# microsoft/rl-offline-simulation

Hardware: AMD Instinct MI355X
Metric: simulated steps/sec (node), 10M logged transitions x 4096 rollouts (higher is better)
Workload: dtype f64

## Files before the change

include/offsim.h:

```cpp
#ifndef OFFSIM_H
#define OFFSIM_H

#include <stdint.h>

#ifdef __cplusplus
extern "C" {
#endif

#define OFFSIM_OK 0
#define OFFSIM_EINVAL (-1)
#define OFFSIM_EHIP (-2)
#define OFFSIM_EUNSUPPORTED (-3)

#define OFFSIM_F32 0
#define OFFSIM_F64 1
#define OFFSIM_F16 2

#define OFFSIM_REJECT_DEFAULT 0
#define OFFSIM_REJECT_NEVER 1

#define OFFSIM_PROB_F64 0
#define OFFSIM_PROB_F32 1

#define OFFSIM_ST_OK 0
// ... 1 lines not shown
#define OFFSIM_ST_NO_INIT 2
#define OFFSIM_ST_KEYERROR 3
#define OFFSIM_ST_INACTIVE 4
#define OFFSIM_ST_PROTOCOL 5

typedef struct offsim_table {
    int64_t N;
    int32_t n_slots;
    int32_t nA;
    int32_t plog_dtype;
    int32_t r_dtype;
    const uint32_t *seg_off;
    const void *p_log;
    const int32_t *a;
    const void *r;
    const int32_t *z_next;
    const uint8_t *done;
    const int32_t *orig_idx;
    int64_t N0;
    const int32_t *init_slot;
    const int32_t *init_orig;
    int64_t max_seg;
    int64_t min_seg;
} offsim_table;

typedef struct offsim_rollouts {
    int32_t R;
    uint64_t *rng;
    uint32_t *cursor;
    uint32_t *init_cursor;
    int32_t *cur_slot;
    const uint32_t *perm;
    int64_t perm_stride;
    const uint32_t *init_perm;
    int64_t init_stride;
    int32_t rng_kind;
} offsim_rollouts;
#define OFFSIM_STREAM_PCG64 0
#define OFFSIM_STREAM_PHILOX 1

const char *offsim_last_error(void);
int offsim_version(void);
int offsim_device_count(void);


int64_t offsim_group_scratch_bytes(int64_t N, int32_t n_slots);
int offsim_group_by_state(const int32_t *slot, int64_t N, int32_t n_slots, uint32_t *seg_off ,
                          int32_t *order , void *scratch, void *stream);

int offsim_gather_rows(const void *src, const int32_t *order, int64_t N, int32_t row_bytes, void *dst, void *stream);


int offsim_seed_streams(const uint64_t *seeds, int32_t R, uint64_t *rng_out , void *stream);

int offsim_shuffle_queues(const offsim_table *t, const uint64_t *seeds, int32_t n_perm, uint32_t *perm_out,
                          uint32_t *init_perm_out, void *stream);

int offsim_env_reset(const offsim_table *t, offsim_rollouts *ro, const uint8_t *mask, int32_t *out_init_row,
                     void *stream);


int offsim_step_batch(const offsim_table *t, offsim_rollouts *ro, const void *p_new, int32_t prob_mode,
                      int32_t reject_mode, int32_t advance, int32_t *out_row, int32_t *out_status,
                      uint32_t *out_popped, void *stream);

#define OFFSIM_MAILBOX_MAX_ACTIONS 24
#define OFFSIM_SERVER_CMD_STEP 1
#define OFFSIM_SERVER_CMD_POP_ONE 2
#define OFFSIM_SERVER_CMD_EXIT 3
#define OFFSIM_SERVER_CMD_RESET 4
#define OFFSIM_SERVER_STARTING 1
#define OFFSIM_SERVER_RUNNING 2
#define OFFSIM_SERVER_EXITED 3
typedef struct offsim_step_mailbox {
    uint32_t seq_in;
    uint32_t cmd;
    int32_t reject_mode;
    uint32_t reserved0;
    double p_head[5];
    uint32_t reserved1;
    uint32_t seq_in2;
    double p_tail[OFFSIM_MAILBOX_MAX_ACTIONS - 5];
    uint32_t reserved2[2];
    uint32_t seq_out;
    int32_t row;
    int32_t status;
    uint32_t popped;
    uint32_t state;
    uint32_t reserved3[3];
} offsim_step_mailbox;
int offsim_host_alloc(int64_t bytes, void **host_ptr);
int offsim_host_free(void *host_ptr);
int offsim_step_server_start(const offsim_table *t, offsim_rollouts *ro, offsim_step_mailbox *mailbox, int32_t prob_mode,
                             uint32_t idle_polls, void *stream);
#define OFFSIM_SERVER_GONE 1
#define OFFSIM_SERVER_ANSWER_SECONDS 10.0
int offsim_step_server_call(offsim_step_mailbox *mailbox, const void *p_new, int32_t n_actions, int32_t prob_mode, uint32_t cmd,
                            int32_t reject_mode, uint64_t max_spins, int32_t *out3);

int offsim_env_set_state(offsim_rollouts *ro, const int32_t *slot, const uint8_t *mask, void *stream);

typedef struct {
    const void *src;
    void *dst;
    int64_t row_bytes;
    int32_t zero_if_not_ok;
// ... 246 lines not shown
```

rl-offline-simulation_amd/_lib.py:

```python
import ctypes as C
import os

_HERE = os.path.dirname(os.path.abspath(__file__))
LIB_PATH = os.environ.get("OFFSIM_LIB") or os.path.join(_HERE, "csrc", "liboffsim_hip.so")

OK = 0
EINVAL, EHIP, EUNSUPPORTED = -1, -2, -3
F32, F64, F16 = 0, 1, 2
REJECT_DEFAULT, REJECT_NEVER = 0, 1
STREAM_PCG64, STREAM_PHILOX = 0, 1
STREAMS_A, STREAMS_B, STREAMS_C = 0, 1, 2
PROB_F64, PROB_F32 = 0, 1
ST_OK, ST_EXHAUSTED, ST_NO_INIT, ST_KEYERROR, ST_INACTIVE, ST_PROTOCOL = 0, 1, 2, 3, 4, 5

_vp, _i32, _i64, _u8 = C.c_void_p, C.c_int32, C.c_int64, C.c_uint8


class Table(C.Structure):
    _fields_ = [("N", _i64), ("n_slots", _i32), ("nA", _i32), ("plog_dtype", _i32), ("r_dtype", _i32),
                ("seg_off", _vp), ("p_log", _vp), ("a", _vp), ("r", _vp), ("z_next", _vp), ("done", _vp),
                ("orig_idx", _vp), ("N0", _i64), ("init_slot", _vp), ("init_orig", _vp), ("max_seg", _i64), ("min_seg", _i64)]


class Rollouts(C.Structure):
# ... 61 lines not shown
                ("x_dtype", _i32), ("dO", _i32), ("x_start", _vp), ("x_next", _vp), ("x_init", _vp), ("v_next", _vp), ("v_init", _vp)]


class CollectPPOOut(C.Structure):
    _fields_ = [("value", _vp), ("logp", _vp), ("final_value", _vp), ("v_trunc", _vp)]


PPO_ACTOR, PPO_CRITIC = 0, 1
PPO_MAX_BLOCKS = 256


def ppo_update_work_doubles(P):
    return PPO_MAX_BLOCKS * 8 + 8 + PPO_MAX_BLOCKS * ((P + 1) // 2)


class PPONet(C.Structure):
    _fields_ = [("n_layers", _i32), ("activation", _i32), ("layers_host", C.POINTER(MLPLayer)), ("slope", C.c_float), ("reserved", _i32)]


class PPOBatchC(C.Structure):
    _fields_ = [("obs", _vp), ("x_dtype", _i32), ("dO", _i32), ("act", _vp), ("adv", _vp), ("logp", _vp), ("ret", _vp), ("valid", _vp),
                ("M", _i64)]


class PPOAdam(C.Structure):
    _fields_ = [("m", _vp), ("v", _vp), ("t", _vp), ("lr", C.c_double)]


MAILBOX_MAX_ACTIONS = 24
SERVER_CMD_STEP, SERVER_CMD_POP_ONE, SERVER_CMD_EXIT, SERVER_CMD_RESET = 1, 2, 3, 4
SERVER_STARTING, SERVER_RUNNING, SERVER_EXITED = 1, 2, 3
SERVER_GONE = 1
SERVER_ANSWER_SECONDS = 10.0


class StepMailbox(C.Structure):
    _fields_ = [("seq_in", C.c_uint32), ("cmd", C.c_uint32), ("reject_mode", _i32), ("reserved0", C.c_uint32), ("p_head", C.c_double * 5),
                ("reserved1", C.c_uint32), ("seq_in2", C.c_uint32), ("p_tail", C.c_double * (MAILBOX_MAX_ACTIONS - 5)),
                ("reserved2", C.c_uint32 * 2), ("seq_out", C.c_uint32), ("row", _i32), ("status", _i32), ("popped", C.c_uint32),
                ("state", C.c_uint32), ("reserved3", C.c_uint32 * 3)]


TD_QLEARN, TD_EXPSARSA = 1, 2
BEHAVIOUR_FIXED, BEHAVIOUR_EPS_GREEDY, BEHAVIOUR_SOFT_GREEDY = 0, 1, 2

SIGNATURES = {
    "offsim_last_error": (C.c_char_p, []),
    "offsim_version": (C.c_int, []),
    "offsim_device_count": (C.c_int, []),
    "offsim_group_scratch_bytes": (_i64, [_i64, _i32]),
    "offsim_group_by_state": (C.c_int, [_vp, _i64, _i32, _vp, _vp, _vp, _vp]),
    "offsim_gather_rows": (C.c_int, [_vp, _vp, _i64, _i32, _vp, _vp]),
    "offsim_seed_streams": (C.c_int, [_vp, _i32, _vp, _vp]),
    "offsim_shuffle_queues": (C.c_int, [C.POINTER(Table), _vp, _i32, _vp, _vp, _vp]),
    "offsim_env_reset": (C.c_int, [C.POINTER(Table), C.POINTER(Rollouts), _vp, _vp, _vp]),
    "offsim_env_set_state": (C.c_int, [C.POINTER(Rollouts), _vp, _vp, _vp]),
    "offsim_vector_gather": (C.c_int, [_vp, _vp, _vp, C.c_int32, _vp, C.c_int32, _vp, _vp]),
    "offsim_vector_step": (C.c_int, [C.POINTER(Table), C.POINTER(Rollouts), _vp, _i32, _i32, _vp, _i32, _vp, _i32, _vp, _vp, _vp, _vp]),
    "offsim_step_batch": (C.c_int, [C.POINTER(Table), C.POINTER(Rollouts), _vp, _i32, _i32, _i32, _vp, _vp, _vp, _vp]),
    "offsim_eval_mc": (C.c_int, [C.POINTER(Table), C.POINTER(Rollouts), _vp, _i32, _i32, C.c_double, _vp, _i64, _i64,
                                 C.POINTER(EvalMCOut), _vp]),
    "offsim_step_exo": (C.c_int, [C.POINTER(Table), C.POINTER(Table), C.POINTER(Rollouts), C.POINTER(Rollouts), _vp, _i32,
                                  _vp, _vp, _vp, _vp, _vp]),
    "offsim_eval_td": (C.c_int, [C.POINTER(Table), C.POINTER(Rollouts), _vp, _i32, C.c_double, _vp, _i64, _i64,
                                 C.POINTER(EvalMCOut), C.POINTER(TD), _vp]),
    "offsim_compile_policy": (C.c_int, [C.POINTER(Table), _vp, _vp, _vp]),
    "offsim_eval_mc_keys_kernel": (C.c_char_p, [_i32, _i32]),
    "offsim_compile_digests": (C.c_int, [C.POINTER(Table), _vp, _i32, _vp, _vp]),
    "offsim_shuffle_queues_keys": (C.c_int, [C.POINTER(Table), _vp, _i32, _vp, _i32, _vp, _vp, _vp, _vp]),
    "offsim_shuffle_queues_keys_ws": (C.c_int, [C.POINTER(Table), _vp, _i32, _vp, _i32, _vp, _vp, _vp, _vp, _i64, _vp]),
    "offsim_shuffle_workspace_bytes": (_i64, [C.POINTER(Table), _i32]),
    "offsim_shuffle_queues_ws": (C.c_int, [C.POINTER(Table), _vp, _i32, _vp, _vp, _vp, _i64, _vp]),
    "offsim_eval_mc_streams": (C.c_int, [C.POINTER(Table), C.POINTER(Rollouts), C.POINTER(Streams), _vp, C.c_double, _vp, _i64, _i64,
                                         C.POINTER(EvalMCOut), _vp]),
    "offsim_eval_mc_keys": (C.c_int, [C.POINTER(Table), C.POINTER(Rollouts), _vp, C.c_double, _vp, _i64, _i64,
                                      C.POINTER(EvalMCOut), _vp]),
    "offsim_selftest_lds_atomic_order": (C.c_int, [_vp, _vp]),
    "offsim_lds_order_ok": (C.c_int, []),
    "offsim_host_alloc": (C.c_int, [_i64, C.POINTER(_vp)]),
    "offsim_host_free": (C.c_int, [_vp]),
    "offsim_step_server_start": (C.c_int, [C.POINTER(Table), C.POINTER(Rollouts), _vp, _i32, C.c_uint32, _vp]),
    "offsim_step_server_call": (C.c_int, [_vp, _vp, _i32, _i32, C.c_uint32, _i32, C.c_uint64, _vp]),
    "offsim_async_faults": (C.c_int, []),
    "offsim_encode_box": (C.c_int, [_vp, _i64, _vp, _vp]),
    "offsim_encode_mlp": (C.c_int, [_vp, _i32, _i64, _i32, _vp, _vp, _i32, _vp, _vp, _i32, _vp, _vp, _vp]),
    "offsim_eval_mc_rows_policy": (C.c_int, [C.POINTER(Table), C.POINTER(Rollouts), _vp, _vp, _i32, _i32, C.c_double, _vp, _i64, _i64,
                                             C.POINTER(EvalMCOut), _vp, _vp]),
    "offsim_policy_mlp": (C.c_int, [_vp, _i32, _i64, _i32, _vp, _i64, C.POINTER(MLPLayer), _i32, _i32, C.c_float, _vp, _vp]),
    "offsim_vector_collect": (C.c_int, [C.POINTER(Table), C.POINTER(Rollouts), C.POINTER(CollectPolicy), _i32, _i32, _i64, _i32,
                                        C.POINTER(CollectState), C.POINTER(CollectOut), _vp]),
    "offsim_value_mlp": (C.c_int, [_vp, _i32, _i64, _i32, _vp, _i64, C.POINTER(MLPLayer), _i32, _i32, C.c_float, _vp, _vp]),
    "offsim_vector_collect_ppo": (C.c_int, [C.POINTER(Table), C.POINTER(Rollouts), C.POINTER(CollectPolicy), C.POINTER(CollectValue), _i32, _i32,
                                            _i64, _i32, C.POINTER(CollectState), C.POINTER(CollectOut), C.POINTER(CollectPPOOut), _vp]),
    "offsim_ppo_advantages": (C.c_int, [_vp, _vp, _vp, _vp, _vp, _i64, _i64, C.c_double, C.c_double, _i32, _vp, _vp, _vp, _vp, _vp, _vp]),
    "offsim_ppo_update_work_doubles": (_i64, [C.POINTER(PPONet)]),
    "offsim_ppo_grad": (C.c_int, [C.POINTER(PPONet), _i32, C.POINTER(PPOBatchC), C.c_double, _vp, _vp, _vp, _vp]),
    "offsim_ppo_update": (C.c_int, [C.POINTER(PPONet), _i32, C.POINTER(PPOBatchC), C.c_double, C.c_double, _i32, C.POINTER(PPOAdam), _vp, _vp,
                                    _vp, _vp]),
}

_lib = None


class OffsimError(RuntimeError):
    pass

# ... 73 lines not shown
```

rl-offline-simulation_amd/csrc/offsim_hip.hip:

```cpp
#include <hip/hip_fp16.h>
#include <hip/hip_runtime.h>
#include <mutex>
#include <stdint.h>
#include <stdio.h>
#include <stdlib.h>
#include <string.h>
#include <time.h>

#include "offsim.h"
#include "discount.hpp"
#include "pcg64_dev.hpp"
#include "philox_dev.hpp"

extern "C" int offsim_lds_order_ok(void);
#include "shuffle_wave.hpp"
#include "shuffle_chunk.hpp"

using namespace offsim;

static thread_local char g_err[512] = "";

static int fail(int code, const char *fmt, const char *detail = "") {
    snprintf(g_err, sizeof(g_err), fmt, detail);
    return code;
// ... 123 lines not shown
    hipLaunchKernelGGL(k_group_scan_slots, dim3(1), dim3(WAVE), 0, st, totals, n_slots, seg_off);
    LAUNCH_CHECK();
    hipLaunchKernelGGL(k_group_scatter, dim3((unsigned)n_chunks), dim3(WAVE), lds, st, slot, N, n_slots, hist, seg_off, order);
    LAUNCH_CHECK();
    return OFFSIM_OK;
}

template <typename T>
__global__ void k_gather_elem(const T *__restrict__ src, const int32_t *__restrict__ order, int64_t N, T *__restrict__ dst) {
    int64_t g = (int64_t)blockIdx.x * blockDim.x + threadIdx.x;
    if (g < N) dst[g] = src[order[g]];
}
template <typename W>
__global__ void k_gather_words(const W *__restrict__ src, const int32_t *__restrict__ order, int64_t N, int32_t words, W *__restrict__ dst) {
    int64_t i = (int64_t)blockIdx.x * blockDim.x + threadIdx.x;
    if (i >= N * words) return;
    int64_t g = i / words;
    int32_t w = (int32_t)(i - g * words);
    dst[i] = src[(int64_t)order[g] * words + w];
}
extern "C" int offsim_gather_rows(const void *src, const int32_t *order, int64_t N, int32_t row_bytes, void *dst, void *stream) {
    if (N < 0 || row_bytes <= 0) return fail(OFFSIM_EINVAL, "gather_rows: bad argument%s");
    if (N == 0) return OFFSIM_OK;
    hipStream_t st = (hipStream_t)stream;
    unsigned nb = (unsigned)((N + 255) / 256);
    if (row_bytes == 1) hipLaunchKernelGGL(k_gather_elem<uint8_t>, dim3(nb), dim3(256), 0, st, (const uint8_t *)src, order, N, (uint8_t *)dst);
    else if (row_bytes == 2) hipLaunchKernelGGL(k_gather_elem<uint16_t>, dim3(nb), dim3(256), 0, st, (const uint16_t *)src, order, N, (uint16_t *)dst);
    else if (row_bytes == 4) hipLaunchKernelGGL(k_gather_elem<uint32_t>, dim3(nb), dim3(256), 0, st, (const uint32_t *)src, order, N, (uint32_t *)dst);
    else if (row_bytes == 8) hipLaunchKernelGGL(k_gather_elem<uint64_t>, dim3(nb), dim3(256), 0, st, (const uint64_t *)src, order, N, (uint64_t *)dst);
    else {
        const int32_t wb = row_bytes % 4 == 0 ? 4 : row_bytes % 2 == 0 ? 2 : 1, words = row_bytes / wb;
        unsigned nbw = (unsigned)((N * words + 255) / 256);
        if (wb == 4) hipLaunchKernelGGL(k_gather_words<uint32_t>, dim3(nbw), dim3(256), 0, st, (const uint32_t *)src, order, N, words, (uint32_t *)dst);
        else if (wb == 2) hipLaunchKernelGGL(k_gather_words<uint16_t>, dim3(nbw), dim3(256), 0, st, (const uint16_t *)src, order, N, words, (uint16_t *)dst);
        else hipLaunchKernelGGL(k_gather_words<uint8_t>, dim3(nbw), dim3(256), 0, st, (const uint8_t *)src, order, N, words, (uint8_t *)dst);
    }
    LAUNCH_CHECK();
    return OFFSIM_OK;
}

__global__ void k_seed_streams(const uint64_t *__restrict__ seeds, int32_t R, uint64_t *__restrict__ out) {
    int r = blockIdx.x * blockDim.x + threadIdx.x;
    if (r >= R) return;
    PcgInit p = pcg_seed(seeds[r]);
    out[4 * r + 0] = p.state.hi;
    out[4 * r + 1] = p.state.lo;
    out[4 * r + 2] = p.inc.hi;
    out[4 * r + 3] = p.inc.lo;
}
extern "C" int offsim_seed_streams(const uint64_t *seeds, int32_t R, uint64_t *rng_out, void *stream) {
    if (R < 0 || !seeds || !rng_out) return fail(OFFSIM_EINVAL, "seed_streams: bad argument%s");
    if (R == 0) return OFFSIM_OK;
    hipLaunchKernelGGL(k_seed_streams, dim3((R + 255) / 256), dim3(256), 0, (hipStream_t)stream, seeds, R, rng_out);
    LAUNCH_CHECK();
    return OFFSIM_OK;
}

static hipError_t allow_big_lds_fn(const void *fn, int bytes) {
    struct Seen {
        const void *fn;
        int max_bytes;
        uint64_t devs;
    };
    static thread_local Seen seen[64];
    static thread_local int n_seen = 0;
    int dev = 0;
    hipError_t e = hipGetDevice(&dev);
    if (e != hipSuccess) return e;
    Seen *hit = nullptr;
    for (int i = 0; i < n_seen; i++)
        if (seen[i].fn == fn) hit = &seen[i];
    if (hit && dev < 64 && bytes <= hit->max_bytes && ((hit->devs >> dev) & 1ull)) return hipSuccess;
    const int want = hit && hit->max_bytes > bytes ? hit->max_bytes : bytes;
    e = hipFuncSetAttribute(fn, hipFuncAttributeMaxDynamicSharedMemorySize, want);
    if (e != hipSuccess) return e;
    if (!hit && n_seen < 64) {
        hit = &seen[n_seen++];
        hit->fn = fn;
        hit->max_bytes = 0;
        hit->devs = 0;
    }
    if (hit) {
        if (want > hit->max_bytes) {
            hit->max_bytes = want;
            hit->devs = 0;
        }
        if (dev < 64) hit->devs |= 1ull << dev;
    }
    return hipSuccess;
}
#define allow_big_lds(kernel, bytes) allow_big_lds_fn((const void *)(kernel), (bytes))

template <int K>
static int shuf_launch_cuts(int n_launches, size_t lds_top, unsigned n_blocks, hipStream_t st, const offsim_table *t, const uint64_t *seeds, int32_t n_perm,
                            uint32_t *perm_out, uint32_t *init_perm_out, uint32_t lo, uint32_t hi, const uint32_t *dig32, uint32_t *dig_out,
                            uint16_t *loc_out, uint32_t a_xchg) {
    constexpr uint32_t TOP = K == 0 ? 0u : shuf_cuts[K > 0 ? K - 1 : 0], STOP = K == shuf_n_cuts ? 1u : shuf_cuts[K < shuf_n_cuts ? K : 0];
    constexpr uint32_t SQ = K == 0 ? SHUF_SQ_BIG : SHUF_SQ_SMALL;
    if (K >= n_launches) return OFFSIM_OK;
    const size_t ldsb = K == 0 ? lds_top : shuf_fixed_lds_bytes(SQ) + (size_t)TOP * 2 + 16;
    HIP_TRY(allow_big_lds((k_shuffle_wave<true, SQ, TOP, STOP>), 160 * 1024));
    hipLaunchKernelGGL((k_shuffle_wave<true, SQ, TOP, STOP>), dim3(n_blocks), dim3(256), ldsb, st, t->seg_off, t->n_slots, t->N, t->N0, seeds, n_perm,
                       perm_out, init_perm_out, lo, hi, dig32, dig_out, loc_out, a_xchg);
    LAUNCH_CHECK();
    if constexpr (K < shuf_n_cuts)
        return shuf_launch_cuts<K + 1>(n_launches, lds_top, n_blocks, st, t, seeds, n_perm, perm_out, init_perm_out, lo, hi, dig32, dig_out, loc_out, a_xchg);
// ... 1841 lines not shown
```

rl-offline-simulation_amd/csrc/pcg64_dev.hpp:

```cpp
#pragma once
#include <hip/hip_runtime.h>
#include <stdint.h>

namespace offsim {

struct U128 {
    uint64_t lo, hi;
};

__device__ __forceinline__ U128 u128(uint64_t hi, uint64_t lo) {
    U128 r;
    r.lo = lo;
    r.hi = hi;
    return r;
}
__device__ __forceinline__ U128 mul128(U128 a, U128 b) {
    U128 r;
    r.lo = a.lo * b.lo;
    r.hi = __umul64hi(a.lo, b.lo) + a.hi * b.lo + a.lo * b.hi;
    return r;
}
__device__ __forceinline__ U128 add128(U128 a, U128 b) {
    U128 r;
    r.lo = a.lo + b.lo;
    r.hi = a.hi + b.hi + (r.lo < a.lo ? 1ull : 0ull);
    return r;
}

#define OFFSIM_PCG_MULT_HI 0x2360ED051FC65DA4ull
#define OFFSIM_PCG_MULT_LO 0x4385DF649FCCF645ull

__device__ __forceinline__ U128 pcg_mult() { return u128(OFFSIM_PCG_MULT_HI, OFFSIM_PCG_MULT_LO); }

__device__ __forceinline__ U128 pcg_step(U128 s, U128 inc) { return add128(mul128(s, pcg_mult()), inc); }

__device__ __forceinline__ uint64_t pcg_output(U128 s) {
    uint64_t x = s.hi ^ s.lo;
    unsigned rot = (unsigned)(s.hi >> 58);
    return (x >> rot) | (x << ((64u - rot) & 63u));
}

struct Jump {
    U128 mult, plus;
};
__device__ inline Jump pcg_jump(U128 inc, uint64_t delta) {
    U128 acc_m = u128(0, 1), acc_p = u128(0, 0);
    U128 cur_m = pcg_mult(), cur_p = inc;
    while (delta > 0) {
        if (delta & 1) {
            acc_m = mul128(acc_m, cur_m);
            acc_p = add128(mul128(acc_p, cur_m), cur_p);
        }
        cur_p = mul128(add128(cur_m, u128(0, 1)), cur_p);
        cur_m = mul128(cur_m, cur_m);
        delta >>= 1;
    }
    Jump j;
    j.mult = acc_m;
    j.plus = acc_p;
    return j;
}
__device__ __forceinline__ U128 pcg_apply(Jump j, U128 s) { return add128(mul128(j.mult, s), j.plus); }

struct PcgInit {
    U128 state, inc;
};
__device__ inline PcgInit pcg_seed(uint64_t seed) {
    const uint32_t MULT_A = 0x931e8875u, MULT_B = 0x58f38dedu, MIX_L = 0xca01f9ddu, MIX_R = 0x4973f715u;
    uint32_t hc = 0x43b0d7e5u;
    uint32_t pool[4];
    uint32_t e1 = (uint32_t)(seed >> 32);
#pragma unroll
    for (int i = 0; i < 4; i++) {
        uint32_t v = (i == 0) ? (uint32_t)seed : ((i == 1 && e1 != 0) ? e1 : 0u);
        v ^= hc;
        hc *= MULT_A;
        v *= hc;
        v ^= v >> 16;
        pool[i] = v;
    }
#pragma unroll
    for (int s = 0; s < 4; s++) {
#pragma unroll
        for (int d = 0; d < 4; d++) {
            if (s != d) {
                uint32_t v = pool[s];
                v ^= hc;
                hc *= MULT_A;
                v *= hc;
                v ^= v >> 16;
                uint32_t m = MIX_L * pool[d] - MIX_R * v;
                m ^= m >> 16;
                pool[d] = m;
            }
        }
    }
    uint32_t hb = 0x8b51f9ddu;
    uint32_t w[8];
#pragma unroll
    for (int i = 0; i < 8; i++) {
        uint32_t v = pool[i & 3];
        v ^= hb;
        hb *= MULT_B;
        v *= hb;
        v ^= v >> 16;
        w[i] = v;
    }
    uint64_t q0 = (uint64_t)w[0] | ((uint64_t)w[1] << 32), q1 = (uint64_t)w[2] | ((uint64_t)w[3] << 32);
    uint64_t q2 = (uint64_t)w[4] | ((uint64_t)w[5] << 32), q3 = (uint64_t)w[6] | ((uint64_t)w[7] << 32);
    PcgInit r;
    r.inc = u128((q2 << 1) | (q3 >> 63), (q3 << 1) | 1ull);
    U128 s = u128(0, 0);
    s = pcg_step(s, r.inc);
    s = add128(s, u128(q0, q1));
    s = pcg_step(s, r.inc);
    r.state = s;
    return r;
}

struct PcgSeq {
    U128 state, inc;
    uint32_t hi32;
    bool has32;
    __device__ __forceinline__ void init(PcgInit p) {
        state = p.state;
        inc = p.inc;
        has32 = false;
        hi32 = 0;
    }
    __device__ __forceinline__ uint64_t next64() {
        state = pcg_step(state, inc);
        return pcg_output(state);
    }
    __device__ __forceinline__ uint32_t next32() {
        if (has32) {
            has32 = false;
            return hi32;
        }
        uint64_t n = next64();
        has32 = true;
        hi32 = (uint32_t)(n >> 32);
        return (uint32_t)n;
    }
    __device__ __forceinline__ uint32_t interval32(uint32_t max) {
        uint32_t mask = 0xffffffffu >> __clz((int)max);
        uint32_t v;
        do {
            v = next32() & mask;
        } while (v > max);
        return v;
    }
};

}
```

rl-offline-simulation_amd/csrc/shuffle_chunk.hpp:

```cpp
#pragma once
#include <hip/hip_runtime.h>
#include <stdint.h>

#include "pcg64_dev.hpp"
#include "shuffle_wave.hpp"

namespace offsim {

enum { SC_WORK = 11, SC_NCH = 12 };

__host__ __device__ inline uint32_t shc_list_cap(uint32_t n, uint32_t lo, uint32_t hi) {
#ifdef SHC_TEST_SMALL_LISTS
    return 16u;
#endif
    if (hi >= n) return 128u;
    const float mu = (float)(hi - lo) * logf((float)n / (float)hi);
    return (uint32_t)(mu + 8.0f * sqrtf(mu)) + 128u;
}
__device__ __forceinline__ void shc_touch(const void *gptr, uint32_t lds_dst_uniform) {
    uint32_t keep;
    asm volatile(
        "s_mov_b32 %0, m0\n\t"
        "s_mov_b32 m0, %2\n\t"
        "s_nop 0\n\t"
// ... 43 lines not shown
    lds_vu32 *xd = rcnt + kcap;
    lds_vu32 *xl = xd + (PLAIN ? 0u : CB + 64u);
    const int wave = __builtin_amdgcn_readfirstlane(threadIdx.x >> 6), lane = threadIdx.x & 63;
    uint64_t *m64 = ws + (int64_t)blockIdx.x * ws_block_words;
    uint32_t *m32 = (uint32_t *)(m64 + msg_cap);
    uint64_t *rpool = m64 + msg_cap + (PLAIN ? 0u : (msg_cap + 1u) / 2u);
    unsigned char *lc_plain = (unsigned char *)(m64 + ws_block_words - lc_words);
    const uint32_t n_work = n_work_seg[0] * (uint32_t)n_perm;

    for (;;) {
        __syncthreads();
        if (threadIdx.x == 0) ctrl[SC_WORK] = atomicAdd(counter, 1u);
        __syncthreads();
        const uint32_t w = ctrl[SC_WORK];
        if (w >= n_work) return;
        const uint32_t s = work_seg[w / (uint32_t)n_perm];
        const int32_t r = (int32_t)(w % (uint32_t)n_perm);
        const bool initq = s == (uint32_t)n_slots, plain = initq || perm_out != nullptr;
        const uint32_t beg = initq ? 0u : seg_off[s], n = initq ? (uint32_t)N0 : seg_off[s + 1] - beg;
        const uint32_t K = (n + CB - 1u) / CB;
        uint32_t *dg = initq ? init_perm + (int64_t)r * N0 : (perm_out ? perm_out : dig_out) + (int64_t)r * N + beg;
        unsigned char *lc = plain ? lc_plain : (unsigned char *)loc_out + ((int64_t)r * N + beg) * (int64_t)(loc_bits >> 3);
        const uint32_t base_val = initq ? 0u : beg;
        const uint32_t *dsrc = plain ? seg_off : dig32 + beg;
        __syncthreads();
        if (threadIdx.x < 16u) ctrl[threadIdx.x] = 0u;
        for (uint32_t k = threadIdx.x; k < K; k += 256u) {
            const uint32_t lo = k * CB, hi = lo + CB < n ? lo + CB : n;
            moff[k + 1u] = shc_list_cap(n, lo, hi);
            mcnt[k] = 0u;
            rcnt[k] = 0u;
        }
        __syncthreads();
        if (threadIdx.x == 0) {
            uint32_t off = 0;
            for (uint32_t k = 0; k < K; k++) {
                const uint32_t cap = moff[k + 1u];
                moff[k] = off;
                off += cap;
            }
            moff[K] = off;
            if (off > msg_cap) {
                ctrl[SH_ABORT] = 1u;
                atomicOr(&g_async_fault, OFFSIM_FAULT_SHUFFLE);
            }
        }
        __syncthreads();
        if (ctrl[SH_ABORT]) return;

        if (n >= 2u) {
            if (wave == 0 || wave == 3) {
                const uint32_t g = wave == 0 ? 0u : 1u;
                const PcgInit p = pcg_seed(seeds[r]);
                const Jump j128 = pcg_jump(p.inc, 128);
                U128 st = pcg_apply(pcg_jump(p.inc, 64ull * g + (uint64_t)lane + 1), p.state);
                uint32_t blk = g, done_blocks = 0, cpub = 0;
                for (;;) {
                    bool stop = false;
                    uint32_t polls = 0;
                    while ((blk + 1u) * 128u - cpub > SHC_RG) {
                        shuf_bound(ctrl, polls);
                        if (sh_ld(ctrl + SH_DONE)) {
                            stop = true;
                            break;
                        }
                        __builtin_amdgcn_s_sleep(2);
                        cpub = sh_ld(ctrl + SH_CPUB);
                    }
                    if (stop) break;
                    const uint64_t o = pcg_output(st);
                    st = pcg_apply(j128, st);
                    const uint32_t idx = (blk * 128u + 2u * (uint32_t)lane) & (SHC_RG - 1u);
#ifdef SHUF_G_B64
                    *(lds_vu64 *)(ring + idx) = o;
#else
                    ring[idx] = (uint32_t)o;
                    ring[idx + 1u] = (uint32_t)(o >> 32);
#endif
                    blk += 2u;
                    done_blocks++;
                    sh_st(ctrl + (g ? SH_GEN1 : SH_GEN0), done_blocks);
                }
            } else if (wave == 1) {
                uint32_t i = n - 1u, c = 0, avail = 0, fill = 0, tail = 0, c_pub = 0;
                uint32_t mask = 0xffffffffu >> __builtin_clz(i);
                int lowpow = (int)((mask >> 1) + 1u);
                auto wait_draws = [&](uint32_t upto) {
                    uint32_t polls = 0;
                    while (upto > avail) {
                        const uint64_t gg = *(lds_vu64 *)(ctrl + SH_GEN0);
                        const uint32_t g0 = sh_rfl((uint32_t)gg), g1 = sh_rfl((uint32_t)(gg >> 32));
                        avail = 128u * (g0 <= g1 ? 2u * g0 : 2u * g1 + 1u);
                        if (upto > avail) {
                            shuf_bound(ctrl, polls);
                            __builtin_amdgcn_s_sleep(1);
                        }
                    }
                };
                auto wait_room = [&](uint32_t upto) {
                    uint32_t polls = 0;
                    while (upto - tail > SHC_SQ) {
                        tail = sh_ld(ctrl + SH_TAIL);
                        if (upto - tail > SHC_SQ) {
                            shuf_bound(ctrl, polls);
                            __builtin_amdgcn_s_sleep(2);
                        }
                    }
                };
// ... 334 lines not shown
```

rl-offline-simulation_amd/csrc/shuffle_wave.hpp:

```cpp
#pragma once
#include <type_traits>
#include <hip/hip_runtime.h>
#include <stdint.h>

#include "pcg64_dev.hpp"

namespace offsim {

#define SHUF_RG 2048u
#ifndef SHUF_CUT_LIST
#define SHUF_CUT_LIST 32768u, 8192u, 2048u
#endif
constexpr uint32_t shuf_cuts[] = {SHUF_CUT_LIST};
constexpr int shuf_n_cuts = (int)(sizeof(shuf_cuts) / sizeof(shuf_cuts[0]));
constexpr bool shuf_cuts_ok() {
    for (int k = 0; k < shuf_n_cuts; k++)
        if ((shuf_cuts[k] & (shuf_cuts[k] - 1u)) != 0u || shuf_cuts[k] < 1024u || (k == 0 ? shuf_cuts[k] > 32768u : shuf_cuts[k] >= shuf_cuts[k - 1])) return false;
    return true;
}
static_assert(shuf_cuts_ok(), "SHUF_CUT_LIST: descending powers of two, 32768 at most, 1024 at least");
#define SHUF_SQ_BIG 4096u
#define SHUF_SQ_SMALL 1024u
#define SHUF_CAP16 65536u
enum { SH_GEN0 = 0, SH_GEN1 = 1, SH_CPUB = 2, SH_FILL = 3, SH_TAIL = 4, SH_DONE = 5, SH_ATOP = 6, SH_EM0 = 7, SH_EM1 = 8, SH_CSTOP = 9,
       SH_ABORT = 10 };
__device__ int32_t g_async_fault = 0;
#define SHUF_SPIN_LIMIT (1u << 20)
__device__ __noinline__ void shuf_bound_check(volatile __attribute__((address_space(3))) uint32_t *ctrl, uint32_t polls) {
    if (polls > SHUF_SPIN_LIMIT) ctrl[SH_ABORT] = 1u;
    if (ctrl[SH_ABORT]) {
        if ((threadIdx.x & 63u) == 0u) atomicOr(&g_async_fault, OFFSIM_FAULT_SHUFFLE);
        __builtin_amdgcn_endpgm();
    }
}
__device__ __forceinline__ void shuf_bound(volatile __attribute__((address_space(3))) uint32_t *ctrl, uint32_t &polls) {
#ifndef SHUF_NO_BOUND
    if (__builtin_expect((++polls & 1023u) == 0u, 0)) shuf_bound_check(ctrl, polls);
#endif
}
#define SHUF_CH 512u

typedef __attribute__((address_space(3))) volatile uint32_t lds_vu32;
typedef __attribute__((address_space(3))) volatile uint16_t lds_vu16;
typedef __attribute__((address_space(3))) volatile uint64_t lds_vu64;

__device__ __forceinline__ uint32_t sh_rfl(uint32_t v) { return (uint32_t)__builtin_amdgcn_readfirstlane(v); }
__device__ __forceinline__ uint32_t sh_ld(lds_vu32 *p) { return sh_rfl(*p); }
__device__ __forceinline__ void sh_st(lds_vu32 *p, uint32_t v) { *p = v; }
__device__ __forceinline__ uint64_t sh_lowmask(uint32_t k) { return k >= 64u ? ~0ull : ((1ull << k) - 1ull); }
__device__ __forceinline__ uint32_t sh_ff1(uint64_t m) { return (uint32_t)__ffsll((unsigned long long)m) - 1u; }
__device__ __forceinline__ int sh_rank(uint64_t m) {
    return (int)__builtin_amdgcn_mbcnt_hi((uint32_t)(m >> 32), __builtin_amdgcn_mbcnt_lo((uint32_t)m, 0u));
}

template <uint32_t TOP>
__device__ __forceinline__ void shuf_fill_from_stream(lds_vu16 *x16, const uint16_t *lc) {
    typedef uint32_t u32x4_a4 __attribute__((ext_vector_type(4), aligned(4)));
    typedef uint32_t u32x4 __attribute__((ext_vector_type(4)));
    constexpr uint32_t VEC = TOP / 8u, J = VEC ? (VEC + 255u) / 256u : 1u;
    static_assert(TOP % 8u == 0u, "the fill moves 16 bytes at a time");
    const bool odd = (((uintptr_t)lc >> 1) & 1u) != 0u;
    const uint32_t *src = (const uint32_t *)(lc - (odd ? 1 : 0));
    __attribute__((address_space(3))) u32x4 *dst = (__attribute__((address_space(3))) u32x4 *)x16;
    u32x4 w[J];
    if (odd) {
        uint32_t e[J];
#pragma unroll
        for (uint32_t j = 0; j < J; j++) {
            const uint32_t q = threadIdx.x + 256u * j;
            if (VEC % 256u == 0u || q < VEC) {
                w[j] = *(const u32x4_a4 *)(src + 4u * q);
                e[j] = src[4u * q + 4u];
            }
        }
        __builtin_amdgcn_sched_barrier(0);
#pragma unroll
        for (uint32_t j = 0; j < J; j++) {
            const uint32_t q = threadIdx.x + 256u * j;
            if (VEC % 256u == 0u || q < VEC) {
                u32x4 o;
                o.x = __builtin_amdgcn_alignbyte(w[j].y, w[j].x, 2u);
                o.y = __builtin_amdgcn_alignbyte(w[j].z, w[j].y, 2u);
                o.z = __builtin_amdgcn_alignbyte(w[j].w, w[j].z, 2u);
                o.w = __builtin_amdgcn_alignbyte(e[j], w[j].w, 2u);
                dst[q] = o;
            }
        }
    } else {
#pragma unroll
        for (uint32_t j = 0; j < J; j++) {
            const uint32_t q = threadIdx.x + 256u * j;
            if (VEC % 256u == 0u || q < VEC) w[j] = *(const u32x4_a4 *)(src + 4u * q);
        }
        __builtin_amdgcn_sched_barrier(0);
#pragma unroll
        for (uint32_t j = 0; j < J; j++) {
            const uint32_t q = threadIdx.x + 256u * j;
            if (VEC % 256u == 0u || q < VEC) dst[q] = w[j];
        }
    }
}

constexpr uint32_t shuf_fixed_lds_bytes(uint32_t sq) { return 4u * (16u + SHUF_RG + sq + 64u + 64u); }

template <bool LDS16, uint32_t SHUF_SQ, uint32_t TOP = 0, uint32_t STOP = 1>
__global__ void __launch_bounds__(256)
    k_shuffle_wave(const uint32_t *__restrict__ seg_off, int32_t n_slots, int64_t N, int64_t N0, const uint64_t *__restrict__ seeds,
                   int32_t n_perm, uint32_t *__restrict__ perm, uint32_t *__restrict__ init_perm, uint32_t n_lo, uint32_t n_hi,
                   const uint32_t *__restrict__ dig32, uint32_t *__restrict__ dig_out, uint16_t *__restrict__ loc_out, uint32_t a_xchg) {
    extern __shared__ __align__(16) unsigned char lds_raw[];
    lds_vu32 *ctrl = (lds_vu32 *)lds_raw;
    lds_vu32 *ring = ctrl + 16;
    lds_vu32 *jq = ring + SHUF_RG;
    lds_vu32 *win = jq + SHUF_SQ + 64u;
    lds_vu16 *x16 = (lds_vu16 *)(win + 64u);
#ifdef SHUF_PROF
    const uint64_t pf_entry = __builtin_amdgcn_s_memtime();
#endif
    const int wave = __builtin_amdgcn_readfirstlane(threadIdx.x >> 6), lane = threadIdx.x & 63;

    const int32_t s_idx = (int32_t)(blockIdx.x / (uint32_t)n_perm);
    const int32_t r = (int32_t)(blockIdx.x - (uint32_t)s_idx * (uint32_t)n_perm);
    const int32_t s = s_idx == 0 ? n_slots : s_idx - 1;
    uint32_t n, base_val;
    uint32_t *xg;
    if (s < n_slots) {
        const uint32_t b = seg_off[s];
        n = seg_off[s + 1] - b;
        xg = perm + (int64_t)r * N + b;
        base_val = b;
    } else {
        n = (uint32_t)N0;
        xg = init_perm + (int64_t)r * N0;
        base_val = 0;
    }
    if (n == 0) return;
    if (n <= n_lo || (LDS16 && n > n_hi)) return;
    volatile uint32_t *x32 = (volatile uint32_t *)xg;
    constexpr bool FROM_STREAM = TOP != 0u, CUT = STOP > 1u;
    static_assert(!(FROM_STREAM || CUT) || LDS16, "the cut form is for LDS-resident keyed chains");
    static_assert((TOP & (TOP - 1u)) == 0u && (STOP & (STOP - 1u)) == 0u && (TOP == 0u || TOP > STOP), "cuts are powers of two");
    if ((FROM_STREAM || CUT) && (dig_out == nullptr || s >= n_slots)) return;
    const uint32_t n_rows = n;
    if (FROM_STREAM) n = TOP;
    const uint32_t stop_i = STOP;

    const bool keyed = LDS16 && dig_out != nullptr && s < n_slots;
    const uint32_t *dsrc = keyed ? dig32 + base_val : nullptr;
    uint32_t *dg = keyed ? dig_out + (int64_t)r * N + base_val : nullptr;
    uint16_t *lc = keyed ? loc_out + (int64_t)r * N + base_val : nullptr;
    const uint32_t n_chunks = (n + SHUF_CH - 1u) / SHUF_CH;
    auto emit_chunk = [&](uint32_t ch) {
        lds_vu32 *xw = (lds_vu32 *)x16;
        const uint32_t pairs = (n + 1u) >> 1, k0 = ch * (SHUF_CH / 2u) + (uint32_t)lane;
        uint32_t two[4], d0[4], d1[4];
#pragma unroll
        for (int u = 0; u < 4; u++) {
            const uint32_t k = k0 + 64u * (uint32_t)u;
            two[u] = k < pairs ? xw[k] : 0u;
        }
        if (CUT && ch < STOP / SHUF_CH) {
#pragma unroll
            for (int u = 0; u < 4; u++) {
                const uint32_t k = k0 + 64u * (uint32_t)u;
                lc[2u * k] = (uint16_t)(two[u] & 0xffffu);
                lc[2u * k + 1u] = (uint16_t)(two[u] >> 16);
            }
            return;
        }
#pragma unroll
        for (int u = 0; u < 4; u++) {
            const uint32_t i1 = two[u] >> 16;
            d0[u] = dsrc[two[u] & 0xffffu];
            d1[u] = dsrc[i1 < n_rows ? i1 : 0u];
        }
#pragma unroll
        for (int u = 0; u < 4; u++) {
            const uint32_t k = k0 + 64u * (uint32_t)u;
            if (k < pairs) {
                dg[2u * k] = d0[u];
                lc[2u * k] = (uint16_t)(two[u] & 0xffffu);
                if (2u * k + 1u < n) {
                    dg[2u * k + 1u] = d1[u];
                    lc[2u * k + 1u] = (uint16_t)(two[u] >> 16);
                }
            }
        }
    };

    if (threadIdx.x < 16u) ctrl[threadIdx.x] = threadIdx.x == SH_ATOP ? n - 1u : (threadIdx.x == SH_EM0 || threadIdx.x == SH_EM1) ? n_chunks : 0u;
    if (threadIdx.x < 64u) win[threadIdx.x] = 0;
    uint32_t c_start = 0;
    if (FROM_STREAM) {
        c_start = dg[0];
        shuf_fill_from_stream<TOP>(x16, lc);
    } else if (LDS16) {
        __attribute__((address_space(3))) uint32_t *xw = (__attribute__((address_space(3))) uint32_t *)x16;
        for (uint32_t k = threadIdx.x; 2u * k < n; k += 256u) xw[k] = ((2u * k + 1u) << 16) | (2u * k);
    } else {
        for (uint32_t k = threadIdx.x; k < n; k += 256u) xg[k] = base_val + k;
    }
    __syncthreads();

#ifdef SHUF_PROF
    uint64_t pf_wait = 0, pf_w0 = 0, pf_extra = 0, pf_g_first = 0;
    const uint64_t pf_begin = __builtin_amdgcn_s_memtime();
#define SPW0() pf_w0 = __builtin_amdgcn_s_memtime()
#define SPW1() pf_wait += __builtin_amdgcn_s_memtime() - pf_w0
#define SPX1() pf_extra += __builtin_amdgcn_s_memtime() - pf_w0
#else
#define SPW0()
#define SPW1()
#define SPX1()
#endif
    if (n >= 2) {
        if (wave == 0 || wave == 3) {
            const uint32_t g = wave == 0 ? 0u : 1u;
            const PcgInit p = pcg_seed(seeds[r]);
            const Jump j128 = pcg_jump(p.inc, 128);
            U128 st = pcg_apply(pcg_jump(p.inc, (uint64_t)(c_start >> 1) + 64ull * g + (uint64_t)lane + 1), p.state);
            uint32_t blk = g, done_blocks = 0, cpub = 0;
            int32_t em_next = (int32_t)n_chunks - 1 - (int32_t)(((n_chunks - 1u) & 1u) != g);
            for (;;) {
                bool stop = false;
                SPW0();
                uint32_t polls = 0;
                while ((blk + 1u) * 128u - cpub > SHUF_RG) {
                    shuf_bound(ctrl, polls);
                    if (sh_ld(ctrl + SH_DONE)) {
                        stop = true;
                        break;
                    }
                    if (keyed && em_next >= 0 && sh_ld(ctrl + SH_ATOP) < SHUF_CH * (uint32_t)em_next) {
#ifdef SHUF_PROF
                        const uint64_t e0 = __builtin_amdgcn_s_memtime();
                        emit_chunk((uint32_t)em_next);
                        pf_extra += __builtin_amdgcn_s_memtime() - e0;
#else
                        emit_chunk((uint32_t)em_next);
#endif
                        sh_st(ctrl + (g ? SH_EM1 : SH_EM0), (uint32_t)em_next);
                        em_next -= 2;
                    } else {
                        __builtin_amdgcn_s_sleep(1);
                    }
                    cpub = sh_ld(ctrl + SH_CPUB);
                }
                SPW1();
                if (stop) break;
                const uint64_t o = pcg_output(st);
                st = pcg_apply(j128, st);
                const uint32_t idx = (blk * 128u + 2u * (uint32_t)lane) & (SHUF_RG - 1u);
                *(lds_vu64 *)(ring + idx) = o;
                blk += 2u;
                done_blocks++;
                sh_st(ctrl + (g ? SH_GEN1 : SH_GEN0), done_blocks);
#ifdef SHUF_PROF
                if (done_blocks == 1u) pf_g_first = __builtin_amdgcn_s_memtime() - pf_begin;
#endif
            }
        } else if (wave == 1) {
            uint32_t i = n - 1u, c = c_start & 1u, avail = 0, fill = 0, tail = 0;
            uint32_t mask = 0xffffffffu >> __builtin_clz(i);
            int lowpow = (int)((mask >> 1) + 1u);
            auto wait_draws = [&](uint32_t upto) {
                if (__builtin_expect(upto <= avail, 1)) return;
                const bool waited = upto > avail;
                if (waited) SPW0();
                uint32_t polls = 0;
                while (upto > avail) {
                    const uint64_t gg = *(lds_vu64 *)(ctrl + SH_GEN0);
                    const uint32_t g0 = sh_rfl((uint32_t)gg), g1 = sh_rfl((uint32_t)(gg >> 32));
                    avail = 128u * (g0 <= g1 ? 2u * g0 : 2u * g1 + 1u);
// ... 438 lines not shown
```

Before: 16.19 billion.

## Replace PCG jump-ahead loops with compile-time jump tables and overlap with LDS fill

Replaces the runtime pcg_jump computations, which used a log-step loop of 128-bit multiplies, with constexpr tables of precomputed jump multipliers and increment sums. It adds a per-lane table for the lane offsets and a 6-level base-64 digit table for arbitrary counts. The chain start is moved ahead of the LDS fill so the RNG setup overlaps the global loads of the stream fill. A probe kernel is added to check table-based results against the reference jumps. Risks are added constant-memory lookups and register pressure from hoisting state across the fill.

```diff
diff --git a/include/offsim.h b/include/offsim.h
--- a/include/offsim.h
+++ b/include/offsim.h
@@ -77,6 +77,10 @@
 
 
 int offsim_seed_streams(const uint64_t *seeds, int32_t R, uint64_t *rng_out , void *stream);
+
+#define OFFSIM_PCG_PROBE_WORDS 132
+int offsim_pcg_jump_probe(const uint64_t *seeds, int32_t n_seeds, const uint32_t *counts, int32_t n_counts, int32_t halve,
+                          uint64_t *out_tab , uint64_t *out_ref, void *stream);
 
 int offsim_shuffle_queues(const offsim_table *t, const uint64_t *seeds, int32_t n_perm, uint32_t *perm_out,
                           uint32_t *init_perm_out, void *stream);
diff --git a/rl-offline-simulation_amd/_lib.py b/rl-offline-simulation_amd/_lib.py
--- a/rl-offline-simulation_amd/_lib.py
+++ b/rl-offline-simulation_amd/_lib.py
@@ -137,6 +137,7 @@
     "offsim_group_by_state": (C.c_int, [_vp, _i64, _i32, _vp, _vp, _vp, _vp]),
     "offsim_gather_rows": (C.c_int, [_vp, _vp, _i64, _i32, _vp, _vp]),
     "offsim_seed_streams": (C.c_int, [_vp, _i32, _vp, _vp]),
+    "offsim_pcg_jump_probe": (C.c_int, [_vp, _i32, _vp, _i32, _i32, _vp, _vp, _vp]),
     "offsim_shuffle_queues": (C.c_int, [C.POINTER(Table), _vp, _i32, _vp, _vp, _vp]),
     "offsim_env_reset": (C.c_int, [C.POINTER(Table), C.POINTER(Rollouts), _vp, _vp, _vp]),
     "offsim_env_set_state": (C.c_int, [C.POINTER(Rollouts), _vp, _vp, _vp]),
diff --git a/rl-offline-simulation_amd/csrc/offsim_hip.hip b/rl-offline-simulation_amd/csrc/offsim_hip.hip
--- a/rl-offline-simulation_amd/csrc/offsim_hip.hip
+++ b/rl-offline-simulation_amd/csrc/offsim_hip.hip
@@ -199,6 +199,37 @@
     if (R < 0 || !seeds || !rng_out) return fail(OFFSIM_EINVAL, "seed_streams: bad argument%s");
     if (R == 0) return OFFSIM_OK;
     hipLaunchKernelGGL(k_seed_streams, dim3((R + 255) / 256), dim3(256), 0, (hipStream_t)stream, seeds, R, rng_out);
+    LAUNCH_CHECK();
+    return OFFSIM_OK;
+}
+
+__global__ void __launch_bounds__(64) k_pcg_jump_probe(const uint64_t *seeds, const uint32_t *counts, int32_t n_counts, int32_t halve,
+                                                       uint64_t *out_tab, uint64_t *out_ref) {
+    const uint32_t lane = threadIdx.x, g = blockIdx.x & 1u, ci = (blockIdx.x >> 1) % (uint32_t)n_counts, si = (blockIdx.x >> 1) / (uint32_t)n_counts;
+    const PcgJumpRow lane_row = pcg_lane_row(64u * g + lane + 1u);
+    const uint32_t q = sh_rfl(halve ? counts[ci] >> 1 : counts[ci]);
+    const PcgInit p = pcg_seed(seeds[si]);
+    const U128 st = pcg_chain_start(p, lane_row, q);
+    const Jump j128 = pcg_jump_lane(p.inc, 128u);
+    const U128 st_ref = pcg_apply(pcg_jump(p.inc, (uint64_t)q + 64ull * g + (uint64_t)lane + 1), p.state);
+    const Jump j_ref = pcg_jump(p.inc, 128);
+    uint64_t *ot = out_tab + (int64_t)blockIdx.x * OFFSIM_PCG_PROBE_WORDS, *orf = out_ref + (int64_t)blockIdx.x * OFFSIM_PCG_PROBE_WORDS;
+    ot[2u * lane] = st.hi;
+    ot[2u * lane + 1u] = st.lo;
+    orf[2u * lane] = st_ref.hi;
+    orf[2u * lane + 1u] = st_ref.lo;
+    if (lane == 0) {
+        ot[128] = j128.mult.hi, ot[129] = j128.mult.lo, ot[130] = j128.plus.hi, ot[131] = j128.plus.lo;
+        orf[128] = j_ref.mult.hi, orf[129] = j_ref.mult.lo, orf[130] = j_ref.plus.hi, orf[131] = j_ref.plus.lo;
+    }
+}
+extern "C" int offsim_pcg_jump_probe(const uint64_t *seeds, int32_t n_seeds, const uint32_t *counts, int32_t n_counts, int32_t halve,
+                                     uint64_t *out_tab, uint64_t *out_ref, void *stream) {
+    if (n_seeds < 0 || n_counts < 0 || !seeds || !counts || !out_tab || !out_ref) return fail(OFFSIM_EINVAL, "pcg_jump_probe: bad argument%s");
+    if ((int64_t)n_seeds * n_counts > (1 << 20)) return fail(OFFSIM_EINVAL, "pcg_jump_probe: at most 2^20 {seed, count} pairs%s");
+    if (n_seeds == 0 || n_counts == 0) return OFFSIM_OK;
+    hipLaunchKernelGGL(k_pcg_jump_probe, dim3(2u * (unsigned)n_seeds * (unsigned)n_counts), dim3(64), 0, (hipStream_t)stream, seeds, counts, n_counts, halve,
+                       out_tab, out_ref);
     LAUNCH_CHECK();
     return OFFSIM_OK;
 }
diff --git a/rl-offline-simulation_amd/csrc/pcg64_dev.hpp b/rl-offline-simulation_amd/csrc/pcg64_dev.hpp
--- a/rl-offline-simulation_amd/csrc/pcg64_dev.hpp
+++ b/rl-offline-simulation_amd/csrc/pcg64_dev.hpp
@@ -1,6 +1,8 @@
 #pragma once
 #include <hip/hip_runtime.h>
 #include <stdint.h>
+
+#include "pcg64_jump_tab.hpp"
 
 namespace offsim {
 
@@ -62,6 +64,23 @@
 }
 __device__ __forceinline__ U128 pcg_apply(Jump j, U128 s) { return add128(mul128(j.mult, s), j.plus); }
 
+__device__ __forceinline__ PcgJumpRow pcg_lane_row(uint32_t k) { return g_pcg_lane_tab.row[k - 1u]; }
+__device__ __forceinline__ Jump pcg_jump_from_row(PcgJumpRow w, U128 inc) {
+    Jump j;
+    j.mult = u128(w.a_hi, w.a_lo);
+    j.plus = mul128(u128(w.s_hi, w.s_lo), inc);
+    return j;
+}
+__device__ __forceinline__ Jump pcg_jump_lane(U128 inc, uint32_t k) { return pcg_jump_from_row(pcg_lane_row(k), inc); }
+__device__ __forceinline__ U128 pcg_apply_count(U128 state, U128 inc, uint32_t q) {
+#pragma unroll
+    for (uint32_t lv = 0; lv < OFFSIM_PCG_COUNT_LEVELS; lv++) {
+        const uint32_t d = (q >> (OFFSIM_PCG_COUNT_BITS * lv)) & (uint32_t)OFFSIM_PCG_COUNT_DIGITS;
+        if (d != 0u) state = pcg_apply(pcg_jump_from_row(g_pcg_count_tab.row[lv * OFFSIM_PCG_COUNT_DIGITS + d - 1u], inc), state);
+    }
+    return state;
+}
+
 struct PcgInit {
     U128 state, inc;
 };
@@ -118,6 +137,10 @@
     return r;
 }
 
+__device__ __forceinline__ U128 pcg_chain_start(PcgInit p, PcgJumpRow lane_row, uint32_t q) {
+    return pcg_apply(pcg_jump_from_row(lane_row, p.inc), pcg_apply_count(p.state, p.inc, q));
+}
+
 struct PcgSeq {
     U128 state, inc;
     uint32_t hi32;
diff --git a/rl-offline-simulation_amd/csrc/pcg64_jump_tab.hpp b/rl-offline-simulation_amd/csrc/pcg64_jump_tab.hpp
--- /dev/null
+++ b/rl-offline-simulation_amd/csrc/pcg64_jump_tab.hpp
@@ -0,0 +1,62 @@
+#pragma once
+#include <stdint.h>
+
+namespace offsim {
+
+typedef unsigned __int128 pcg_u128;
+
+struct PcgJumpRow {
+    uint64_t a_lo, a_hi, s_lo, s_hi;
+};
+
+#define OFFSIM_PCG_LANE_ROWS 128
+#define OFFSIM_PCG_COUNT_BITS 6
+#define OFFSIM_PCG_COUNT_LEVELS 6
+#define OFFSIM_PCG_COUNT_DIGITS ((1 << OFFSIM_PCG_COUNT_BITS) - 1)
+#define OFFSIM_PCG_COUNT_ROWS (OFFSIM_PCG_COUNT_LEVELS * OFFSIM_PCG_COUNT_DIGITS)
+
+template <int N>
+struct PcgJumpTab {
+    PcgJumpRow row[N];
+};
+
+constexpr pcg_u128 pcg_tab_mult() { return ((pcg_u128)0x2360ED051FC65DA4ull << 64) | (pcg_u128)0x4385DF649FCCF645ull; }
+constexpr PcgJumpRow pcg_tab_row(pcg_u128 a, pcg_u128 s) {
+    return PcgJumpRow{(uint64_t)a, (uint64_t)(a >> 64), (uint64_t)s, (uint64_t)(s >> 64)};
+}
+
+constexpr PcgJumpTab<OFFSIM_PCG_LANE_ROWS> pcg_make_lane_tab() {
+    PcgJumpTab<OFFSIM_PCG_LANE_ROWS> t{};
+    pcg_u128 a = 1, s = 0;
+    for (int k = 1; k <= OFFSIM_PCG_LANE_ROWS; k++) {
+        s = s * pcg_tab_mult() + 1;
+        a = a * pcg_tab_mult();
+        t.row[k - 1] = pcg_tab_row(a, s);
+    }
+    return t;
+}
+
+constexpr PcgJumpTab<OFFSIM_PCG_COUNT_ROWS> pcg_make_count_tab() {
+    PcgJumpTab<OFFSIM_PCG_COUNT_ROWS> t{};
+    pcg_u128 base_a = pcg_tab_mult(), base_s = 1;
+    for (int lv = 0; lv < OFFSIM_PCG_COUNT_LEVELS; lv++) {
+        pcg_u128 a = 1, s = 0;
+        for (int d = 1; d <= OFFSIM_PCG_COUNT_DIGITS; d++) {
+            s = s * base_a + base_s;
+            a = a * base_a;
+            t.row[lv * OFFSIM_PCG_COUNT_DIGITS + d - 1] = pcg_tab_row(a, s);
+        }
+        base_s = s * base_a + base_s;
+        base_a = a * base_a;
+    }
+    return t;
+}
+
+static_assert(sizeof(PcgJumpTab<OFFSIM_PCG_COUNT_ROWS>) <= 64 * 1024, "the count table stays small enough for the scalar cache's neighbourhood");
+
+#ifdef __HIPCC__
+static __device__ constexpr PcgJumpTab<OFFSIM_PCG_LANE_ROWS> g_pcg_lane_tab = pcg_make_lane_tab();
+static __device__ constexpr PcgJumpTab<OFFSIM_PCG_COUNT_ROWS> g_pcg_count_tab = pcg_make_count_tab();
+#endif
+
+}
diff --git a/rl-offline-simulation_amd/csrc/shuffle_chunk.hpp b/rl-offline-simulation_amd/csrc/shuffle_chunk.hpp
--- a/rl-offline-simulation_amd/csrc/shuffle_chunk.hpp
+++ b/rl-offline-simulation_amd/csrc/shuffle_chunk.hpp
@@ -119,8 +119,8 @@
             if (wave == 0 || wave == 3) {
                 const uint32_t g = wave == 0 ? 0u : 1u;
                 const PcgInit p = pcg_seed(seeds[r]);
-                const Jump j128 = pcg_jump(p.inc, 128);
-                U128 st = pcg_apply(pcg_jump(p.inc, 64ull * g + (uint64_t)lane + 1), p.state);
+                const Jump j128 = pcg_jump_lane(p.inc, 128u);
+                U128 st = pcg_apply(pcg_jump_lane(p.inc, 64u * g + (uint32_t)lane + 1u), p.state);
                 uint32_t blk = g, done_blocks = 0, cpub = 0;
                 for (;;) {
                     bool stop = false;
diff --git a/rl-offline-simulation_amd/csrc/shuffle_wave.hpp b/rl-offline-simulation_amd/csrc/shuffle_wave.hpp
--- a/rl-offline-simulation_amd/csrc/shuffle_wave.hpp
+++ b/rl-offline-simulation_amd/csrc/shuffle_wave.hpp
@@ -53,8 +53,8 @@
     return (int)__builtin_amdgcn_mbcnt_hi((uint32_t)(m >> 32), __builtin_amdgcn_mbcnt_lo((uint32_t)m, 0u));
 }
 
-template <uint32_t TOP>
-__device__ __forceinline__ void shuf_fill_from_stream(lds_vu16 *x16, const uint16_t *lc) {
+template <uint32_t TOP, class MID>
+__device__ __forceinline__ void shuf_fill_from_stream(lds_vu16 *x16, const uint16_t *lc, MID mid) {
     typedef uint32_t u32x4_a4 __attribute__((ext_vector_type(4), aligned(4)));
     typedef uint32_t u32x4 __attribute__((ext_vector_type(4)));
     constexpr uint32_t VEC = TOP / 8u, J = VEC ? (VEC + 255u) / 256u : 1u;
@@ -63,17 +63,20 @@
     const uint32_t *src = (const uint32_t *)(lc - (odd ? 1 : 0));
     __attribute__((address_space(3))) u32x4 *dst = (__attribute__((address_space(3))) u32x4 *)x16;
     u32x4 w[J];
+    uint32_t e[J];
+#pragma unroll
+    for (uint32_t j = 0; j < J; j++) {
+        const uint32_t q = threadIdx.x + 256u * j;
+        e[j] = 0u;
+        if (VEC % 256u == 0u || q < VEC) {
+            w[j] = *(const u32x4_a4 *)(src + 4u * q);
+            if (odd) e[j] = src[4u * q + 4u];
+        }
+    }
+    __builtin_amdgcn_sched_barrier(0);
+    mid();
+    __builtin_amdgcn_sched_barrier(0);
     if (odd) {
-        uint32_t e[J];
-#pragma unroll
-        for (uint32_t j = 0; j < J; j++) {
-            const uint32_t q = threadIdx.x + 256u * j;
-            if (VEC % 256u == 0u || q < VEC) {
-                w[j] = *(const u32x4_a4 *)(src + 4u * q);
-                e[j] = src[4u * q + 4u];
-            }
-        }
-        __builtin_amdgcn_sched_barrier(0);
 #pragma unroll
         for (uint32_t j = 0; j < J; j++) {
             const uint32_t q = threadIdx.x + 256u * j;
@@ -87,12 +90,6 @@
             }
         }
     } else {
-#pragma unroll
-        for (uint32_t j = 0; j < J; j++) {
-            const uint32_t q = threadIdx.x + 256u * j;
-            if (VEC % 256u == 0u || q < VEC) w[j] = *(const u32x4_a4 *)(src + 4u * q);
-        }
-        __builtin_amdgcn_sched_barrier(0);
 #pragma unroll
         for (uint32_t j = 0; j < J; j++) {
             const uint32_t q = threadIdx.x + 256u * j;
@@ -190,14 +187,29 @@
 
     if (threadIdx.x < 16u) ctrl[threadIdx.x] = threadIdx.x == SH_ATOP ? n - 1u : (threadIdx.x == SH_EM0 || threadIdx.x == SH_EM1) ? n_chunks : 0u;
     if (threadIdx.x < 64u) win[threadIdx.x] = 0;
+    const bool is_g = wave == 0 || wave == 3;
+    const uint32_t g = wave == 0 ? 0u : 1u;
     uint32_t c_start = 0;
+    PcgJumpRow lane_row = {0, 0, 0, 0};
+    if (is_g) lane_row = pcg_lane_row(64u * g + (uint32_t)lane + 1u);
+    U128 st = u128(0, 0);
+    Jump j128;
+    j128.mult = j128.plus = u128(0, 0);
+    auto chain_start = [&]() __attribute__((always_inline)) {
+        if (FROM_STREAM) c_start = sh_rfl(dg[0]);
+        if (!is_g) return;
+        const PcgInit p = pcg_seed(seeds[r]);
+        j128 = pcg_jump_lane(p.inc, 128u);
+        st = pcg_chain_start(p, lane_row, c_start >> 1);
+    };
     if (FROM_STREAM) {
-        c_start = dg[0];
-        shuf_fill_from_stream<TOP>(x16, lc);
+        shuf_fill_from_stream<TOP>(x16, lc, chain_start);
     } else if (LDS16) {
+        chain_start();
         __attribute__((address_space(3))) uint32_t *xw = (__attribute__((address_space(3))) uint32_t *)x16;
         for (uint32_t k = threadIdx.x; 2u * k < n; k += 256u) xw[k] = ((2u * k + 1u) << 16) | (2u * k);
     } else {
+        chain_start();
         for (uint32_t k = threadIdx.x; k < n; k += 256u) xg[k] = base_val + k;
     }
     __syncthreads();
@@ -215,10 +227,6 @@
 #endif
     if (n >= 2) {
         if (wave == 0 || wave == 3) {
-            const uint32_t g = wave == 0 ? 0u : 1u;
-            const PcgInit p = pcg_seed(seeds[r]);
-            const Jump j128 = pcg_jump(p.inc, 128);
-            U128 st = pcg_apply(pcg_jump(p.inc, (uint64_t)(c_start >> 1) + 64ull * g + (uint64_t)lane + 1), p.state);
             uint32_t blk = g, done_blocks = 0, cpub = 0;
             int32_t em_next = (int32_t)n_chunks - 1 - (int32_t)(((n_chunks - 1u) & 1u) != g);
             for (;;) {
```

Result: faster. 16.60 billion (median of 6 runs) (+2.5%).
